# tongxyh/ImageCompression_Adversarial

Hardware: AMD Instinct MI355X
Metric: attack-step·images/sec, Balle2018-hyper 768×512 1001-step PGD, 1/2/4/8 GPU (higher is better)
Workload: dtype f32 (fp32-accurate: exact 3-way bf16 operand splits, 6 MFMA products, f32 accumulate); 1 GPU; attack_rd -m hyper -q 3 -att_metric L2 -noise 1e-4, 32 images/GPU of 768x512, steps of the 1001-step loop, x6 conv operands; per_gpu_batch=32, global_batch=32, height=512, width=768, parallelism=image-shard x1 (no data-path collective)

## Files before the change

imagecompression_adversarial_amd/_lib.py:

```python
from __future__ import annotations

import ctypes as C
import os

import torch

_HERE = os.path.dirname(os.path.abspath(__file__))
LIB_PATH = os.environ.get("ICA_HIP_LIB", os.path.join(_HERE, "libica_hip.so"))

_p = C.c_void_p
_i = C.c_int
_l = C.c_long
_f = C.c_float
_sz = C.c_size_t

_SIGS = {
    "ica_conv_it": [_i],
    "ica_pack_conv_weight_size": [_i, _i, _i, _i, _i],
    "ica_pack_conv_weight": [_p, _p, _i, _i, _i, _l, _l, _i, _i, _i, _i, _p],
    "ica_pack_conv_weight_bf16": [_p, _p, _i, _i, _i, _l, _l, _i, _i, _i, _p],
    "ica_pack_conv_weight_bf16_size": [_i, _i, _i, _i],
    "ica_pack_conv_weight_x6": [_p, _p, _i, _i, _i, _l, _l, _i, _i, _p],
    "ica_pack_conv_weight_x6_size": [_i, _i, _i, _i],
    "ica_pack_gdn_x6": [_p, _p, _i, _p],
    "ica_pack_gdn_x6_size": [_i],
    "ica_pack_up3_bf16": [_p, _p, _i, _p],
    "ica_pack_up3_x6": [_p, _p, _i, _p],
    "ica_pack_up3k3_x6_size": [_i],
    "ica_pack_up3k3_x6": [_p, _p, _p, _i, _p],
    "ica_conv_up3k3_x6": [_p, _p, _p, _p, _i, _i, _i, _i, _i, _i, _p],
    "ica_conv_up3_x6": [_p, _p, _p, _p, _i, _i, _i, _i, _i, _p],
    "ica_conv_up3_bf16": [_p, _p, _p, _p, _i, _i, _i, _i, _i, _p],
    "ica_conv_ex": [_p, _p],
    "ica_last_launch": [_p, _i, _p],
    "ica_pack_gdn": [_p, _p, _p, _p, _i, _i, _f, _p],
    "ica_pack_gdn_bf16": [_p, _p, _p, _p, _i, _i, _f, _p],
    "ica_pack_up3_size": [_i],
    "ica_pack_up3": [_p, _p, _i, _p],
    "ica_conv_up3": [_p, _p, _p, _p, _i, _i, _i, _i, _i, _p],
    "ica_elem_blocks_per_image": [],
    "ica_nchw_to_nc4": [_p, _p, _i, _i, _i, _i, _p],
    "ica_nc4_to_nchw": [_p, _p, _i, _i, _i, _i, _p],
    "ica_reduce_rows": [_p, _p, _i, _i, _f, _p],
    "ica_attack_prologue": [_p, _p, _p, _p, _i, _i, _i, _f, _p],
    "ica_attack_prologue_ex": [_p, _p, _p, _p, _i, _i, _i, _f, _i, _p],
    "ica_attack_loss": [_p, _p, _p, _p, _i, _i, _i, _f, _i, _i, _p],
    "ica_attack_adam": [_p, _p, _p, _p, _p, _p, _p, _p, _i, _i, _i, _f, _f, _f, _f, _f, _p, _p, _p, _p],
    "ica_attack_adam_ex": [_p, _p, _p, _p, _p, _p, _p, _p, _i, _i, _i, _f, _f, _f, _f, _f, _p, _p, _p, _i, _p],
# ... 73 lines not shown
    "ica_eb_bwd": [_p, _p, _p, _p, _p, _i, _i, _i, _i, _p],
    "ica_eb_param_scatter": [_p, _p, _p, _i, _p],
    "ica_mse_grad": [_p, _p, _p, _i, _i, _i, _f, _p],
}
_RESTYPES = {"ica_pack_conv_weight_size": _sz, "ica_pack_conv_weight_bf16_size": _sz,
             "ica_pack_conv_weight_x6_size": _sz, "ica_pack_gdn_x6_size": _sz, "ica_pack_up3k3_x6_size": _sz, "ica_pack_up3_size": _sz, "ica_wgrad_ws_size": _sz,
             "ica_rans_encode": _l, "ica_ar_lds_bytes": _sz, "ica_patch_vi_ws_size": _sz,
             "ica_gauss_blur_ws_size": _sz, "ica_blur_sweep_ws_size": _sz, "ica_noise_apply_ws_size": _sz}



class ConvArgs(C.Structure):
    _fields_ = ([(n, C.c_void_p) for n in ("x", "y", "wp", "bias", "gp", "beta", "save_x", "save_s", "in_x", "in_s",
                                            "save_t", "res", "mask")]
                + [(n, C.c_int) for n in ("N", "Cin", "Hin", "Win", "Cout", "Hout", "Wout", "kind", "KS", "S", "epi",
                                           "it", "fill_mode", "ps", "prec", "layout", "order")])


class ArArgs(C.Structure):
    _fields_ = ([(n, C.c_void_p) for n in ("y", "params", "yhat", "sym", "idx", "sym_in", "means", "wc", "bc", "w1",
                                            "b1", "w2", "b2", "w3", "b3", "table")]
                + [("T", C.c_int), ("bound", C.c_float)]
                + [(n, C.c_int) for n in ("B", "M", "H", "W", "E1", "E2")])


_lib = None


def lib():
    global _lib
    if _lib is None:
# ... 32 lines not shown
```

imagecompression_adversarial_amd/csrc/ica_conv.hip:

```cpp
#include <cxxabi.h>

#include <algorithm>
#include <cstdio>
#include <cstdlib>
#include <type_traits>

#include "ica_conv_epi.h"

#define ICA_WLOAD_BF(w, it, g) ((w)[(it) * 64])

template <int IT, int KH>
ICA_DEV void load_frag(float (&a)[IT][KH], const float* w) {
#pragma unroll
  for (int it = 0; it < IT; ++it) {
    if constexpr (KH == 8) {
      const f32x4 w0 = ld4(w + it * 64 * KH), w1 = ld4(w + it * 64 * KH + 4);
#pragma unroll
      for (int e = 0; e < 4; ++e) {
        a[it][e] = w0[e];
        a[it][4 + e] = w1[e];
      }
    } else {
      const f32x2 w0 = *reinterpret_cast<const f32x2*>(w + it * 64 * KH);
      a[it][0] = w0[0];
// ... 1381 lines not shown
              o2 += zs[(2 * 25 + tap) * NPX + q];
            }
          o[px] = f32x4{o0 + bias0, o1 + bias1, o2 + bias2, 0.f};
        }
        const int y = 2 * a + py, x = 2 * b;
        float* dst = p.y + (((size_t)n * p.Hout + y) * p.Wout + x) * 4;
        if (y < p.Hout) {
          st4(dst, o[0]);
          if (x + 1 < p.Wout) st4(dst + 4, o[1]);
        }
      }
    }
  }
}

__global__ void pack_up3_x6_kernel(const float* __restrict__ w, __bf16* __restrict__ dst, int Cin, long total) {
  const long i = (long)blockIdx.x * blockDim.x + threadIdx.x;
  if (i >= total) return;
  const int nch = Cin / 16;
  long t = i;
  const int s = t % 8; t /= 8;
  const int lane = t % 64; t /= 64;
  const int ch = t % nch; t /= nch;
  const int row = (int)t * 32 + (lane & 31);
  const int c = ch * 16 + (lane >> 5) * 8 + s;
  float v = 0.f;
  if (row < T3_ROWS) v = w[((size_t)c * 3 + row / 25) * 25 + row % 25];
  const __bf16 a = (__bf16)v;
  const float r1 = v - (float)a;
  const __bf16 b = (__bf16)r1;
// ... 454 lines not shown
  const float* bias;
  const float* gp;
  const float* beta;
  float* save_x;
  float* save_s;
  const float* in_x;
  const float* in_s;
  float* save_t;
  const float* res;
  const float* mask;
  int N, Cin, Hin, Win, Cout, Hout, Wout;
  int kind, KS, S, epi, it, fill_mode, ps;
  int prec;
  int layout;
  int order;
} ica_conv_args;

int ica_conv_it(int cout) {
  if (cout <= 32) return 1;
  if (cout % 128 == 0) return 4;
  if (cout % 96 == 0) return 3;
  return 4;
}

static inline int resolve_it(int O, int it) { return it > 0 ? it : ica_conv_it(O); }

size_t ica_pack_conv_weight_size(int O, int C, int KS, int CC, int it) {
  const int IT = resolve_it(O, it);
  const int ncb = (O + IT * 32 - 1) / (IT * 32);
  const int C4 = (C + 3) / 4, nch = (C4 * 4 + CC - 1) / CC;
// ... 106 lines not shown
               N, Cin, Hin, Win, 3, 2 * Hin, 2 * Win, nullptr};
  p.pl = layout;
  auto persistent = [&](auto kern, int R) {
    const int tiles = ((Win + U3_OW - 1) / U3_OW) * ((Hin + R - 1) / R) * N;
    const int nb = std::max(1, std::min((tiles + 7) / 8, ica_cu_count() / 8));
    ICA_LAUNCH(kern, dim3(8 * nb), dim3(256), 0, st, p);
  };
  if (Cin == 128) {
    persistent(conv_up3_x6p_kernel<8, 3>, u3_rows<3>());
  } else if (Cin == 192) {
    persistent(conv_up3_x6p_kernel<12, 2>, u3_rows<2>());
  } else {
    const int tiles = ((Win + T3_TW - 1) / T3_TW) * ((Hin + T3_TH - 1) / T3_TH) * N;
    ICA_LAUNCH((conv_up3_kernel<false, true>), dim3(tiles), dim3(256), 0, st, p);
  }
  ICA_CHECK_LAUNCH();
  return 0;
}

int ica_pack_up3_bf16(const float* w, void* dst, int Cin, hipStream_t st) {
  if (Cin % 16 != 0) return -2;
  const long total = (long)ica_pack_up3_size(Cin);
  ICA_LAUNCH(pack_up3_kernel<__bf16>, dim3((total + 255) / 256), dim3(256), 0, st, w,
                     reinterpret_cast<__bf16*>(dst), Cin, total);
  ICA_CHECK_LAUNCH();
  return 0;
}

int ica_conv_up3_bf16(const float* x, float* y, const void* wp, const float* bias, int N, int Cin, int Hin, int Win,
                      int layout, hipStream_t st) {
// ... 63 lines not shown
                     transpose, beta_bound);
  ICA_CHECK_LAUNCH();
  return 0;
}

int ica_conv_ex(const ica_conv_args* a, hipStream_t st) {
  ConvParams p{a->x,    a->y,    a->wp,   a->bias, a->gp,   a->beta, a->save_x, a->save_s, a->in_x, a->in_s,
               a->N,    a->Cin,  a->Hin,  a->Win,  a->Cout, a->Hout, a->Wout,   a->save_t, a->res,  a->mask,
               a->fill_mode, a->ps, a->prec, a->layout};
  if (a->prec < 0 || a->prec > 3) return -4;
  if (a->layout & ~(PL_IN | PL_OUT)) return -4;
  if (a->layout && (a->KS != 5 || a->S != 2 || a->fill_mode != 0 || a->ps)) return -4;
  if (((a->layout & PL_IN) && ((a->Hin | a->Win) & 1)) || ((a->layout & PL_OUT) && ((a->Hout | a->Wout) & 1)))
    return -2;
  const int it = resolve_it(a->Cout, a->it);
  if (a->epi >= EPI_GDN && a->epi <= EPI_IGDN_BWD && a->Cout != it * 32) return -4;
  if (a->ps && (a->Cout % 16 != 0 || !(a->epi == EPI_BIAS || a->epi == EPI_RELU || a->epi == EPI_LRELU))) return -4;
  if (a->fill_mode == 1 && !a->mask) return -4;
  if (a->fill_mode == 2 && a->Cin % 16 != 0) return -2;
  if (a->epi == EPI_LRELU_BWD && !a->in_x) return -4;
  const int fx = ((a->res || a->save_x) ? FX_RES : 0) | (a->ps ? FX_PS : 0) | (a->fill_mode == 1 ? FX_MASK : 0) |
                 (a->fill_mode == 2 ? FX_UNSHUF : 0) | (a->save_t ? FX_T : 0);
  const int want = a->kind == 1 ? ORDER_UP : ORDER_DOWN;
  if (a->prec == 2) {
    if (a->kind == 0 && a->KS == 3)
      return a->order == want ? pick_x6o<3>(p, a->kind, a->KS, a->S, a->epi, it, fx, st) : -4;
    return ica_conv_x6_dispatch(p, a->kind, a->KS, a->S, it, a->epi, fx, a->order, st);
  }
  if (a->prec == 3) return a->order == want ? pick_x6o<1>(p, a->kind, a->KS, a->S, a->epi, it, fx, st) : -4;
  if (a->prec == 1 && a->order == ORDER_RGB5) {
// ... 13 lines not shown
```

imagecompression_adversarial_amd/csrc/ica_conv_epi.h:

```cpp
#pragma once
#include "ica_common.h"

#ifndef ICA_X6_IEEE_GDN
#define ICA_X6_IEEE_GDN 0
#endif

enum {
  EPI_BIAS = 0,
  EPI_RELU = 1,
  EPI_GDN = 2,
  EPI_IGDN = 3,
  EPI_GDN_BWD = 4,
  EPI_IGDN_BWD = 5,
  EPI_LRELU = 6,
  EPI_LRELU_BWD = 7,
};
enum { FX_RES = 1, FX_PS = 2, FX_MASK = 4, FX_UNSHUF = 8, FX_T = 16 };

struct ConvParams {
  const float* x;
  float* y;
  const float* wp;
  const float* bias;
  const float* gp;
  const float* beta;
  float* save_x;
  float* save_s;
  const float* in_x;
  const float* in_s;
  int N, Cin, Hin, Win, Cout, Hout, Wout;
  float* save_t;
  const float* res;
  const float* mask;
  int fill_mode;
  int ps;
  int prec;
  int pl;
};
enum { PL_IN = 1, PL_OUT = 2 };
enum { ORDER_DOWN = 0, ORDER_UP = 1, ORDER_RGB5 = 2, ORDER_TG = 3 };

ICA_DEV void split3(f32x4 v, u32x2& hi, u32x2& mid, u32x2& lo) {
  bf16x4 a, b, c;
#pragma unroll
  for (int e = 0; e < 4; ++e) {
    const __bf16 h = (__bf16)v[e];
    const float r1 = v[e] - (float)h;
    const __bf16 m = (__bf16)r1;
    const float r2 = r1 - (float)m;
    a[e] = h;
    b[e] = m;
    c[e] = (__bf16)r2;
// ... 55 lines not shown
      v[i] = __builtin_bit_cast(f32x4, __builtin_amdgcn_raw_buffer_load_b128(grs, k * 2048 + l * 16, 0, 0));
    } else {
      v[i] = f32x4{0.f, 0.f, 0.f, 0.f};
    }
  }
#pragma unroll
  for (int i = 0; i < NI; ++i) {
    const int e = threadIdx.x + 256 * i;
    if (e < NP + NG) lp[e] = v[i];
  }
}

ICA_DEV unsigned pix_at(int y, int x, int H, int W, bool split) {
  return split ? ((unsigned)((((y & 1) << 1) | (x & 1)) * (H >> 1) + (y >> 1))) * (unsigned)(W >> 1) + (x >> 1)
               : (unsigned)y * W + x;
}

template <int IT, int EPI, int FX, bool BF = false, int X6 = 0, bool LG = false, int EAG = 1>
ICA_DEV void conv_epilogue(const ConvParams& p, f32x16 (&acc)[IT], int n, int oy, int ox,
                           bool valid, int co_base, const f32x4* lp = nullptr, float* lst = nullptr) {
  const int lane = threadIdx.x & 63, h = lane >> 5;
  const int C4o = (p.Cout + 3) >> 2;
  const unsigned plane = (unsigned)p.Hout * p.Wout;
  const unsigned pix = valid ? pix_at(oy, ox, p.Hout, p.Wout, p.pl & PL_OUT) : 0u;
  const size_t img = (size_t)C4o * plane;
  using Img = Img4T<BF>;
  const unsigned vo = h * plane + pix;
  auto so = [&](int u) -> unsigned { return (unsigned)u * plane; };
  const int cu = co_base >> 2;

// ... 299 lines not shown
          for (int s = 0; s < 2; ++s)
            uacc = mfma32bf(LG ? f4_as_bf8(lp[16 * IT + (k0 + s) * 64 + lane]) : ld_bf8(grs, lane * 16, o + s * 2048),
                            th[ct][s], uacc);
        }
        if (valid) {
#pragma unroll
          for (int g = 0; g < 4; ++g) {
            const f32x4 x2 = bf4_to_f4(x2q[jt][g]);
            f32x4 v;
#pragma unroll
            for (int e = 0; e < 4; ++e) v[e] = acc[jt][4 * g + e] + x2[e] * uacc[4 * g + e];
            Y.st(vo, so(jt * 8 + 2 * g), v);
          }
        }
      }
    } else if constexpr (FX == 0 && IT <= 4) {
      f32x16 tt[X6 == 1 ? 1 : IT], xx[IT];
      bf16x8 tq[X6 == 1 ? IT : 1][2][3];
      const unsigned vo_ld = valid ? vo : 0x0FFFFFF0u;
      float tw[8];
      __builtin_amdgcn_sched_barrier(0);
      f32x4 yq[X6 ? IT : 1][4], sq[X6 ? IT : 1][4];
      if constexpr (X6 != 0) {
#pragma unroll
        for (int it = 0; it < IT; ++it)
#pragma unroll
          for (int g = 0; g < 4; ++g) {
            yq[it][g] = IX.ld(vo_ld, so(it * 8 + 2 * g));
            sq[it][g] = IS.ld(vo_ld, so(it * 8 + 2 * g));
          }
        __builtin_amdgcn_sched_barrier(0);
// ... 38 lines not shown
#pragma unroll
          for (int jt = 0; jt < IT; ++jt)
#pragma unroll
            for (int q = 0; q < 3; ++q)
              a[jt][q] = ld_bf8(grs, lane * 16, (((jt * IT + (k >> 1)) * 2 + (k & 1)) * 1024) + q * IT * IT * 2048);
        };
        ldg(ga[0], 0);
#pragma unroll
        for (int k = 0; k < 2 * IT; ++k) {
          if (k + 1 < 2 * IT) ldg(ga[(k + 1) & 1], k + 1);
          __builtin_amdgcn_sched_barrier(0);
#pragma unroll
          for (int jt = 0; jt < IT; ++jt) ux[jt] = mfma_x6(ga[k & 1][jt], tq[k >> 1][k & 1], ux[jt]);
        }
      }
#pragma unroll
      for (int jt = 0; jt < IT; ++jt) {
        __builtin_amdgcn_sched_barrier(0);
        f32x16 uacc = f32x16{0};
#pragma unroll
        for (int ct = 0; ct < IT; ++ct) {
          if constexpr (X6 == 1) {
            if (ct == 0) uacc = ux[jt];
          } else if constexpr (X6 == 2) {
            if (ct % (IT / 2) == 0) {
              const __amdgpu_buffer_rsrc_t grs = uniform_rsrc(p.gp, IT * IT * 6144);
#pragma unroll
              for (int c2 = 0; c2 < IT / 2; ++c2)
#pragma unroll
                for (int s = 0; s < 2; ++s)
// ... 472 lines not shown
```

imagecompression_adversarial_amd/csrc/ica_conv_x6.hip:

```cpp
#include <algorithm>
#include <type_traits>

#include "ica_conv_epi.h"

namespace {

constexpr int X6_PT = 2;
constexpr int XD_TW = 32;
template <int PT>
constexpr int xd_th() { return 4 * PT; }

template <int IT, int EPI, int PT = X6_PT>
__global__ __launch_bounds__(256, 1) void conv_down_x6_kernel(ConvParams p, long ps) {
  ICA_STAMP_BEGIN();
  constexpr int KS = 5, S = 2, PAD = 2, KK = 25, TW = XD_TW, TH = xd_th<PT>();
  constexpr int PR = S * (TH - 1) + KS, PC = S * (TW - 1) + KS, PLANE = PR * PC;
  constexpr int NF = (4 * PLANE + 255) / 256, NB = (NF + 1) / 2;
  __shared__ f32x4 patch[3 * 2 * PLANE];
  const int tiles_x = (p.Wout + TW - 1) / TW, tiles_y = (p.Hout + TH - 1) / TH;
  int bid, cb;
  xcd_block<true>(bid, cb);
  const int tx = bid % tiles_x;
  bid /= tiles_x;
  const int ty = bid % tiles_y;
// ... 2062 lines not shown
  const int total = ((p.Wout + 31) / 32) * p.Hout * p.N;
  const int nblk = std::max(1, std::min(ica_cu_count(), (total + 7) / 8));
  constexpr int lds = rgb5b_lds_bytes<EPI>();
  static_assert(lds <= 160 * 1024, "conv_rgb5_bf16 LDS");
  static bool attr_set = false;
  if (!attr_set) {
    (void)hipFuncSetAttribute(reinterpret_cast<const void*>(&conv_rgb5_bf16_kernel<EPI>),
                              hipFuncAttributeMaxDynamicSharedMemorySize, lds);
    attr_set = true;
  }
  ICA_LAUNCH((conv_rgb5_bf16_kernel<EPI>), dim3(nblk), dim3(512), lds, st, p, nblk);
  ICA_CHECK_LAUNCH();
  return 0;
}

template <int IT, int EPI, int CG, int PT>
int launch_up_x6_pt(const ConvParams& p, hipStream_t st) {
  const int tiles = ((p.Win + XU_TW - 1) / XU_TW) * ((p.Hin + xu_th<PT>() - 1) / xu_th<PT>()) * p.N;
  const int ncb = (p.Cout + IT * 32 - 1) / (IT * 32);
  const long ps = (long)ncb * 25 * (p.Cin / 16) * IT * 64;
  constexpr size_t lds = xu_lds_bytes<CG, PT>();
  static_assert(lds <= 160 * 1024, "conv_up_x6 channel group exceeds LDS");
  static bool attr_set = false;
  if (!attr_set) {
    (void)hipFuncSetAttribute(reinterpret_cast<const void*>(&conv_up_x6_kernel<IT, EPI, CG, PT>),
                              hipFuncAttributeMaxDynamicSharedMemorySize, 160 * 1024);
    attr_set = true;
  }
  ICA_LAUNCH((conv_up_x6_kernel<IT, EPI, CG, PT>), dim3(tiles, ncb), dim3(256), lds, st, p, ps);
  ICA_CHECK_LAUNCH();
  return 0;
}

template <int IT, int EPI, int CG, int PT = 2>
int launch_up_x6w(const ConvParams& p, hipStream_t st) {
  const int tiles = ((p.Win + XU_TW - 1) / XU_TW) * ((p.Hin + xu_th<PT>() - 1) / xu_th<PT>()) * p.N;
  const int ncb = (p.Cout + IT * 32 - 1) / (IT * 32);
  const long ps = (long)ncb * 25 * (p.Cin / 16) * IT * 64;
  constexpr bool BWD = EPI == EPI_GDN_BWD || EPI == EPI_IGDN_BWD;
  constexpr size_t slabs = BWD ? (size_t)8 * 4 * IT * 64 * sizeof(f32x4) : 0;
  constexpr size_t lds = std::max((size_t)xu_lds_bytes<CG, PT>(), slabs);
  static_assert(lds <= 160 * 1024, "conv_up_x6w LDS");
  static bool attr_set = false;
  if (!attr_set) {
// ... 19 lines not shown
  constexpr bool BWD = EPI == EPI_GDN_BWD || EPI == EPI_IGDN_BWD;
#ifdef ICA_UPW_BWD_ALL
  constexpr bool SLAB = BWD && IT == 4;
#else
  constexpr bool SLAB = BWD && IT == 4 && CG == 64;
#endif
  if (x6_round_fill(b1) > x6_round_fill(b2) + 0.15) {
    if constexpr (SLAB) return launch_up_x6w<IT, EPI, CG, 1>(p, st);
    return launch_up_x6_pt<IT, EPI, CG, 1>(p, st);
  }
  if constexpr (SLAB) return launch_up_x6w<IT, EPI, CG, 2>(p, st);
  if constexpr (IT == 4 && !BWD) return launch_up_x6w<IT, EPI, CG>(p, st);
  return launch_up_x6_pt<IT, EPI, CG, X6_PT>(p, st);
}

template <int IT, int FX, int CG, int PT, int KS = 3>
int launch_up3s2_x6_pt(const ConvParams& p, hipStream_t st) {
  const int tiles = ((p.Win + XU_TW - 1) / XU_TW) * ((p.Hin + xu_th<PT>() - 1) / xu_th<PT>()) * p.N;
  const int ncb = (p.Cout + IT * 32 - 1) / (IT * 32);
  const long ps = (long)ncb * KS * KS * (p.Cin / 16) * IT * 64;
  constexpr size_t lds = xu_lds_bytes<CG, PT>();
  static_assert(lds <= 160 * 1024, "conv_up_x6 channel group exceeds LDS");
  static bool attr_set = false;
  if (!attr_set) {
    (void)hipFuncSetAttribute(reinterpret_cast<const void*>(&conv_up_x6_kernel<IT, EPI_BIAS, CG, PT, KS, FX>),
                              hipFuncAttributeMaxDynamicSharedMemorySize, 160 * 1024);
    attr_set = true;
  }
  ICA_LAUNCH((conv_up_x6_kernel<IT, EPI_BIAS, CG, PT, KS, FX>), dim3(tiles, ncb), dim3(256), lds, st, p, ps);
  ICA_CHECK_LAUNCH();
// ... 71 lines not shown
  return 0;
}

int ica_conv_x6_dispatch(const ConvParams& p, int kind, int KS, int S, int it, int epi, int fx, int order,
                         hipStream_t st) {
  const bool rgb = kind == 0 && KS == 5 && S == 2 && p.Cin <= 4;
  if (order != (rgb ? ORDER_RGB5 : kind == 1 ? ORDER_UP : ORDER_DOWN)) return -4;
  if (kind == 1 && KS == 3 && S == 2) return pick_up3s2_x6(p, it, epi, fx, st);
  if (kind == 1 && KS == 1 && S == 2) {
    if (epi != EPI_BIAS || fx != 0 || p.Cout % 32 != 0) return -4;
    if (p.Hout != 2 * p.Hin || p.Wout != 2 * p.Win || (p.pl & (PL_IN | PL_OUT))) return -2;
    if (it == 6 && p.Cin == 192) return launch_up3s2_x6_pt<6, 0, 192, 1, 1>(p, st);
    if (it == 4 && p.Cin == 128) return launch_up3s2_x6_pt<4, 0, 128, 2, 1>(p, st);
    return -3;
  }
  if (KS != 5 || S != 2 || fx != 0) return -4;
  if (p.Cout % 32 != 0) return -4;
  if (kind == 0) {
    if (p.Hout * 2 != p.Hin + (p.Hin & 1) || p.Wout * 2 != p.Win + (p.Win & 1)) return -2;
    if (p.Cin <= 4) {
      if (it != 4 || p.Cin > 3) return -3;
      if (p.pl & PL_IN) return -2;
      switch (epi) {
        case EPI_BIAS: return launch_rgb_x6<EPI_BIAS>(p, st);
        case EPI_GDN: return launch_rgb_x6<EPI_GDN>(p, st);
        case EPI_IGDN_BWD: return launch_rgb_x6<EPI_IGDN_BWD>(p, st);
        default: return -5;
      }
    }
    if (p.Cin < 16) return -2;
// ... 95 lines not shown
```

imagecompression_adversarial_amd/engine.py:

```python
from __future__ import annotations

import torch

from . import hip_ops as K


def _P(sd, prefix, name):
    return sd[f"{prefix}.{name}" if prefix else name]


class Saved(list):

    def __init__(self, items=(), split=(False,) * 5, exact=True):
        super().__init__(items)
        self.split = tuple(split)
        self.exact = exact


def _layout_of(saved):
    if not isinstance(saved, Saved):
        raise TypeError("backward needs the forward's Saved record (keep its type when selecting rows)")
    return saved.split


# ... 39 lines not shown
            p = self.convs[i]
            h, sx, ss = K.conv_down(h, C, p.fwd, p.bias, self.N, 5, 2, K.EPI_GDN, self.gdns[i], save,
                                    tag=f"{self.tag}.{2 * i}.fwd", layout=_lay(lv, i, i + 1))
            saved.append((sx, ss))
            C = self.N
        p = self.convs[3]
        y, _, _ = K.conv_down(h, self.N, p.fwd, p.bias, self.M, 5, 2, K.EPI_BIAS, tag=f"{self.tag}.6.fwd",
                              layout=_lay(lv, 3, 4))
        return y, saved

    def backward(self, gy4, saved):
        lv = _layout_of(saved)
        if not saved.exact:
            raise ValueError("g_a input gradient: image sides must be multiples of 16")
        g, C = gy4, self.M
        for i in (3, 2, 1):
            g, _, _ = K.conv_up(g, C, self.convs[i].bwd, None, self.N, K.EPI_GDN_BWD, self.gdns[i - 1],
                                saved=saved[i - 1], tag=f"{self.tag}.{2 * i}.dgrad", layout=_lay(lv, i + 1, i))
            C = self.N
        gx, _, _ = K.conv_up(g, self.N, self.convs[0].bwd, None, 3, K.EPI_BIAS, tag=f"{self.tag}.0.dgrad",
                             layout=_lay(lv, 1, 0))
        return gx


class Synthesis:

    def __init__(self, sd: dict, prefix: str = "g_s", tag: str = "g_s", prec: int = K.PREC_FP32):
        self.tag = tag
        self.M = _P(sd, prefix, "0.weight").shape[0]
        self.N = _P(sd, prefix, "0.weight").shape[1]
        g6 = 6 if self.N == 192 else 0
        self.convs = [K.PackedConv(_P(sd, prefix, f"{i}.weight"), _P(sd, prefix, f"{i}.bias"), "deconv", 2, prec,
                                   it_fwd=g6 if i < 6 else 0, it_bwd=g6 if i > 0 else 0)
                      for i in (0, 2, 4, 6)]
# ... 187 lines not shown
```

imagecompression_adversarial_amd/hip_ops.py:

```python
from __future__ import annotations

import math

import torch

from ._lib import ConvArgs, call, lib, ptr, stream

EPI_BIAS, EPI_RELU, EPI_GDN, EPI_IGDN, EPI_GDN_BWD, EPI_IGDN_BWD, EPI_LRELU, EPI_LRELU_BWD = range(8)
FILL_PLAIN, FILL_LRELU_MASK, FILL_UNSHUFFLE = range(3)
ORDER_DOWN, ORDER_UP = 0, 1
ORDER_RGB5 = 2
ORDER_TG = 3
ORDER_UP3 = 4
_ORDER_NAME = ("DOWN", "UP", "RGB5", "TG", "UP3")
LAYOUT_IN, LAYOUT_OUT = 1, 2
GDN_BETA_BOUND = float((1e-6 + 2.0 ** -36) ** 0.5)


EVENT_HOOK = None


def _ev_begin(tag, n):
    if EVENT_HOOK is None or tag is None:
        return None
# ... 325 lines not shown
        return _conv3(x4, Cin, wp, bias, Cout, 5, 2, 1, epi, gdn, save, saved, out, tag, save_t, layout, prec, it)
    _check_pack(wp, Cin, 3, 5, 1, prec, it)
    if wp.order != ORDER_UP3:
        raise ValueError(f"conv_up to 3 channels reads the Z-gather pack (ORDER_UP3), not {wp!r}")
    if epi != EPI_BIAS:
        raise RuntimeError("conv_up to 3 channels supports the bias epilogue only")
    N, _, H, W, _ = x4.shape
    y = out if out is not None else empty_nc4(N, 3, 2 * H, 2 * W, x4.device)
    ev = _ev_begin(_prec_note(tag, wp.prec), N)
    call({PREC_BF16: "ica_conv_up3_bf16", PREC_X6: "ica_conv_up3_x6"}.get(wp.prec, "ica_conv_up3"), ptr(x4), ptr(y),
         ptr(wp.data), ptr(bias), N, Cin, H, W, int(layout), stream())
    _ev_end(ev)
    return y, None, None


def conv_ex(x4, Cin, wp: Pack, bias, Cout, KS, S, kind=0, epi=EPI_BIAS, gdn: PackedGDN | None = None, res=None,
            save_x=None, save_s=None, saved=None, save_t=None, mask=None, fill_mode=FILL_PLAIN, ps=False,
            out=None, tag=None, alg_rows=None, layout=0, prec=None, it=0, _flops=True):
    _check_pack(wp, Cin, Cout, KS, kind, prec, it)
    if wp.order == ORDER_UP3:
        raise ValueError(f"{wp!r} is launched by conv_up to 3 channels only")
    if wp.order == ORDER_RGB5 and (epi not in (EPI_BIAS, EPI_GDN, EPI_IGDN_BWD) or fill_mode != FILL_PLAIN or ps
                                   or any(t is not None for t in (res, save_x, save_t, mask))):
        raise ValueError(f"{wp!r}: the dense tap-row pack is read by conv_rgb5 only (bias / GDN / IGDN_BWD epilogue, "
                         f"plain fill, no extra tensors)")
    prec = wp.prec
    N, C4x, H, W, _ = x4.shape
    if fill_mode == FILL_UNSHUFFLE:
        if Cin != 16 * C4x:
            raise RuntimeError("unshuffled conv input: Cin must be 16 * input channel groups")
        H, W = H // 2, W // 2
    Ho, Wo = _out_hw(H, W, KS, S, kind)
    dt = torch.bfloat16 if prec == PREC_BF16 else torch.float32
    if out is not None:
        y = out
    elif ps:
        y = torch.empty((N, Cout // 16, 2 * Ho, 2 * Wo, 4), dtype=dt, device=x4.device)
    else:
        y = empty_nc4(N, Cout, Ho, Wo, x4.device, dt)
    in_x = in_s = None
    if saved is not None:
        in_x, in_s = saved
    gp = None
    if gdn is not None:
        if prec == PREC_BF16:
            gdn.bf16()
            gp = gdn.gpbT if epi in (EPI_GDN_BWD, EPI_IGDN_BWD) else gdn.gpb
        elif prec in (PREC_X6, PREC_B1):
            gdn.x6()
            gp = gdn.gpxT if epi in (EPI_GDN_BWD, EPI_IGDN_BWD) else gdn.gpx
        else:
            gp = gdn.gpT if epi in (EPI_GDN_BWD, EPI_IGDN_BWD) else gdn.gp
    a = ConvArgs(ptr(x4), ptr(y), ptr(wp.data), ptr(bias), ptr(gp), ptr(None if gdn is None else gdn.beta),
                 ptr(save_x), ptr(save_s), ptr(in_x), ptr(in_s), ptr(save_t), ptr(res), ptr(mask), N, Cin, H, W, Cout,
                 Ho, Wo, kind, KS, S, epi, wp.it, fill_mode, int(bool(ps)), prec, int(layout), wp.order)
    import ctypes
    tag = _prec_note(tag, prec)
    ev = _ev_begin(tag, N)
    call("ica_conv_ex", ctypes.c_void_p(ctypes.addressof(a)), stream())
    if ev is not None:
        fl = None
        if _flops:
            px = N * (H * W if kind == 1 else Ho * Wo)
            cin_alg = alg_rows if (fill_mode == FILL_UNSHUFFLE and alg_rows) else Cin
            cout_alg = alg_rows if (ps and alg_rows) else Cout
            fl = 2.0 * cin_alg * cout_alg * KS * KS * px
            if epi in (EPI_GDN, EPI_IGDN, EPI_GDN_BWD, EPI_IGDN_BWD):
                fl += 2.0 * Cout * Cout * N * Ho * Wo
        _ev_end(ev, fl)
    return y
# ... 197 lines not shown
```

include/ica_hip.h:

```cpp
#ifndef ICA_HIP_H
#define ICA_HIP_H

#include <stddef.h>
#include <stdint.h>

#ifdef __cplusplus
extern "C" {
#endif

typedef struct ihipStream_t* hipStream_t;

enum { ICA_EPI_BIAS = 0, ICA_EPI_RELU = 1, ICA_EPI_GDN = 2, ICA_EPI_IGDN = 3, ICA_EPI_GDN_BWD = 4, ICA_EPI_IGDN_BWD = 5 };

int ica_conv_it(int cout);
size_t ica_pack_conv_weight_size(int O, int C, int KS, int CC, int it);
int ica_pack_conv_weight(const float* w, float* dst, int O, int C, int KS, long so, long sc, int CC, int order,
                         int flip, int it, hipStream_t stream);
int ica_pack_gdn(const float* gamma, const float* beta, float* gp, float* beta_eff, int C, int transpose,
                 float beta_bound, hipStream_t stream);
int ica_pack_conv_weight_bf16(const float* w, void* dst, int O, int C, int KS, long so, long sc, int order,
                              int flip, int it, hipStream_t stream);
int ica_pack_gdn_bf16(const float* gamma, const float* beta, void* gpb, float* beta_eff, int C, int transpose,
                      float beta_bound, hipStream_t stream);
int ica_pack_conv_weight_x6(const float* w, void* dst, int O, int C, int KS, long so, long sc, int order, int it,
// ... 51 lines not shown
  const float* wc;
  const float* bc;
  const float* w1;
  const float* b1;
  const float* w2;
  const float* b2;
  const float* w3;
  const float* b3;
  const float* table;
  int T;
  float bound;
  int B, M, H, W, E1, E2;
} ica_ar_args;
size_t ica_ar_lds_bytes(int M, int E1, int E2);
int ica_ar_step(const ica_ar_args* args, int p0, int p1, int mode, hipStream_t stream);
enum { ICA_EPI_LRELU = 6, ICA_EPI_LRELU_BWD = 7 };
enum { ICA_ORDER_DOWN = 0, ICA_ORDER_UP = 1, ICA_ORDER_RGB5 = 2, ICA_ORDER_TG = 3, ICA_ORDER_UP3 = 4 };
typedef struct ica_conv_args {
  const float* x;
  float* y;
  const float* wp;
  const float* bias;
  const float* gp;
  const float* beta;
  float* save_x;
  float* save_s;
  const float* in_x;
  const float* in_s;
  float* save_t;
  const float* res;
  const float* mask;
  int N, Cin, Hin, Win, Cout, Hout, Wout;
  int kind, KS, S, epi, it, fill_mode, ps;
  int prec;
  int layout;
  int order;
} ica_conv_args;
int ica_conv_ex(const ica_conv_args* args, hipStream_t stream);
int ica_last_launch(char* name, int cap, unsigned long long* threads);
size_t ica_pack_up3_size(int Cin);
int ica_pack_up3(const float* w, float* dst, int Cin, hipStream_t stream);
int ica_conv_up3(const float* x, float* y, const float* wp, const float* bias, int N, int Cin, int Hin, int Win,
                 int layout, hipStream_t stream);

int ica_elem_blocks_per_image(void);
int ica_nchw_to_nc4(const float* src, float* dst, int N, int C, int H, int W, hipStream_t stream);
int ica_nc4_to_nchw(const float* src, float* dst, int N, int C, int H, int W, hipStream_t stream);
int ica_reduce_rows(const float* part, float* out, int B, int nblk, float scale, hipStream_t stream);
int ica_attack_prologue(const float* noise, const float* im_s, float* im_in4, float* part, int B, int H, int W,
                        float eps, hipStream_t stream);
int ica_attack_prologue_ex(const float* noise, const float* im_s, float* im_in4, float* part, int B, int H, int W,
                           float eps, int clamp_in, hipStream_t stream);
int ica_attack_loss(const float* xhat4, const float* out_s, float* grad4, float* part, int B, int H, int W,
// ... 108 lines not shown
```

Measured before the change: 1539 attack-step·images/s.

## Fuse final 3-channel dgrad into GDN-backward conv epilogue via Z-gather

The last g_a input-gradient layer (128→3 channels, 5x5 stride-2 transposed) is folded into the epilogue of the preceding GDN-backward conv. After the GDN backward, the epilogue multiplies the 128-channel gradient by the packed 3-channel weights with x6 MFMAs and writes 75 per-tap partial planes Z. A new gather kernel then sums the taps into the 3-channel output and adds the bias. This avoids writing and re-reading the 128-channel intermediate and skips a separate low-occupancy conv. In exchange it adds a 75-plane fp32 scratch tensor, extra register pressure in the epilogue, and scattered stores.

```diff
diff --git a/imagecompression_adversarial_amd/_lib.py b/imagecompression_adversarial_amd/_lib.py
--- a/imagecompression_adversarial_amd/_lib.py
+++ b/imagecompression_adversarial_amd/_lib.py
@@ -32,6 +32,7 @@
     "ica_conv_up3_x6": [_p, _p, _p, _p, _i, _i, _i, _i, _i, _p],
     "ica_conv_up3_bf16": [_p, _p, _p, _p, _i, _i, _i, _i, _i, _p],
     "ica_conv_ex": [_p, _p],
+    "ica_zgather": [_p, _p, _p, _i, _i, _i, _p],
     "ica_last_launch": [_p, _i, _p],
     "ica_pack_gdn": [_p, _p, _p, _p, _i, _i, _f, _p],
     "ica_pack_gdn_bf16": [_p, _p, _p, _p, _i, _i, _f, _p],
@@ -135,7 +136,8 @@
     _fields_ = ([(n, C.c_void_p) for n in ("x", "y", "wp", "bias", "gp", "beta", "save_x", "save_s", "in_x", "in_s",
                                             "save_t", "res", "mask")]
                 + [(n, C.c_int) for n in ("N", "Cin", "Hin", "Win", "Cout", "Hout", "Wout", "kind", "KS", "S", "epi",
-                                           "it", "fill_mode", "ps", "prec", "layout", "order")])
+                                           "it", "fill_mode", "ps", "prec", "layout", "order")]
+                + [("wz", C.c_void_p)])
 
 
 class ArArgs(C.Structure):
diff --git a/imagecompression_adversarial_amd/csrc/ica_conv.hip b/imagecompression_adversarial_amd/csrc/ica_conv.hip
--- a/imagecompression_adversarial_amd/csrc/ica_conv.hip
+++ b/imagecompression_adversarial_amd/csrc/ica_conv.hip
@@ -1419,6 +1419,52 @@
   }
 }
 
+__global__ __launch_bounds__(256) void zgather_kernel(const float* __restrict__ z, float* __restrict__ y,
+                                                       const float* __restrict__ bias, int N, int Hin, int Win) {
+  const int W2 = Win >> 1, H2 = Hin >> 1, M4 = W2 >> 2;
+  const long idx = (long)blockIdx.x * 256 + threadIdx.x;
+  if (idx >= (long)N * Hin * M4 * 2) return;
+  const int pb = (int)(idx & 1);
+  long t = idx >> 1;
+  const int m = (int)(t % M4);
+  t /= M4;
+  const int a = (int)(t % Hin), n = (int)(t / Hin);
+  const size_t plane = (size_t)Hin * Win;
+  const float* zp = z + (size_t)n * T3_ROWS * plane + ((size_t)(((a & 1) << 1) | pb) * H2 + (a >> 1)) * W2 + 4 * m;
+  const float bias0 = bias ? bias[0] : 0.f, bias1 = bias ? bias[1] : 0.f, bias2 = bias ? bias[2] : 0.f;
+  const int Hout = 2 * Hin, Wout = 2 * Win;
+#pragma unroll
+  for (int py = 0; py < 2; ++py) {
+    float* row = y + ((size_t)n * Hout + 2 * a + py) * Wout * 4;
+#pragma unroll
+    for (int px = 0; px < 2; ++px) {
+      f32x4 o0 = {0.f, 0.f, 0.f, 0.f}, o1 = o0, o2 = o0;
+#pragma unroll
+      for (int ky = py; ky < 5; ky += 2)
+#pragma unroll
+        for (int kx = px; kx < 5; kx += 2) {
+          const int tap = ky * 5 + kx;
+          const bool rows_in = ky < 2 ? a + 1 < Hin : (ky < 4 || a > 0);
+          const int cut = kx < 2 ? (pb == 1 && m == M4 - 1 ? 3 : -1) : (kx == 4 && pb == 0 && m == 0 ? 0 : -1);
+          auto term = [&](int c) {
+            f32x4 v = ld4(zp + (c * 25 + tap) * plane);
+#pragma unroll
+            for (int i = 0; i < 4; ++i) v[i] = (!rows_in || i == cut) ? 0.f : v[i];
+            return v;
+          };
+          o0 += term(0);
+          o1 += term(1);
+          o2 += term(2);
+        }
+#pragma unroll
+      for (int i = 0; i < 4; ++i) {
+        const int x = 2 * (2 * (4 * m + i) + pb) + px;
+        st4(row + (size_t)x * 4, f32x4{o0[i] + bias0, o1[i] + bias1, o2[i] + bias2, 0.f});
+      }
+    }
+  }
+}
+
 __global__ void pack_up3_x6_kernel(const float* __restrict__ w, __bf16* __restrict__ dst, int Cin, long total) {
   const long i = (long)blockIdx.x * blockDim.x + threadIdx.x;
   if (i >= total) return;
@@ -1903,6 +1949,7 @@
   int prec;
   int layout;
   int order;
+  const float* wz;
 } ica_conv_args;
 
 int ica_conv_it(int cout) {
@@ -2039,6 +2086,14 @@
     const int tiles = ((Win + T3_TW - 1) / T3_TW) * ((Hin + T3_TH - 1) / T3_TH) * N;
     ICA_LAUNCH((conv_up3_kernel<false, true>), dim3(tiles), dim3(256), 0, st, p);
   }
+  ICA_CHECK_LAUNCH();
+  return 0;
+}
+
+int ica_zgather(const float* z, float* y, const float* bias, int N, int Hin, int Win, hipStream_t st) {
+  if (N <= 0 || Hin <= 0 || Win <= 0 || (Hin & 1) || (Win & 7)) return -2;
+  const long items = (long)N * Hin * (Win >> 3) * 2;
+  ICA_LAUNCH(zgather_kernel, dim3((unsigned)((items + 255) / 256)), dim3(256), 0, st, z, y, bias, N, Hin, Win);
   ICA_CHECK_LAUNCH();
   return 0;
 }
@@ -2132,6 +2187,13 @@
   if (((a->layout & PL_IN) && ((a->Hin | a->Win) & 1)) || ((a->layout & PL_OUT) && ((a->Hout | a->Wout) & 1)))
     return -2;
   const int it = resolve_it(a->Cout, a->it);
+  if (a->epi == EPI_GDN_BWD_Z) {
+    if (a->prec != 2 || a->kind != 1 || a->KS != 5 || a->S != 2 || !a->wz || a->order != ORDER_UP || a->res ||
+        a->save_x || a->save_t || a->ps || a->fill_mode != 0 || a->Cout != 128 || it != 4 || !a->in_x || !a->in_s)
+      return -4;
+    p.wz = a->wz;
+    return ica_conv_x6_dispatch(p, 1, 5, 2, 4, EPI_GDN_BWD, FX_Z, a->order, st);
+  }
   if (a->epi >= EPI_GDN && a->epi <= EPI_IGDN_BWD && a->Cout != it * 32) return -4;
   if (a->ps && (a->Cout % 16 != 0 || !(a->epi == EPI_BIAS || a->epi == EPI_RELU || a->epi == EPI_LRELU))) return -4;
   if (a->fill_mode == 1 && !a->mask) return -4;
diff --git a/imagecompression_adversarial_amd/csrc/ica_conv_epi.h b/imagecompression_adversarial_amd/csrc/ica_conv_epi.h
--- a/imagecompression_adversarial_amd/csrc/ica_conv_epi.h
+++ b/imagecompression_adversarial_amd/csrc/ica_conv_epi.h
@@ -14,8 +14,9 @@
   EPI_IGDN_BWD = 5,
   EPI_LRELU = 6,
   EPI_LRELU_BWD = 7,
+  EPI_GDN_BWD_Z = 8,
 };
-enum { FX_RES = 1, FX_PS = 2, FX_MASK = 4, FX_UNSHUF = 8, FX_T = 16 };
+enum { FX_RES = 1, FX_PS = 2, FX_MASK = 4, FX_UNSHUF = 8, FX_T = 16, FX_Z = 32 };
 
 struct ConvParams {
   const float* x;
@@ -36,6 +37,7 @@
   int ps;
   int prec;
   int pl;
+  const float* wz;
 };
 enum { PL_IN = 1, PL_OUT = 2 };
 enum { ORDER_DOWN = 0, ORDER_UP = 1, ORDER_RGB5 = 2, ORDER_TG = 3 };
@@ -121,6 +123,75 @@
 ICA_DEV unsigned pix_at(int y, int x, int H, int W, bool split) {
   return split ? ((unsigned)((((y & 1) << 1) | (x & 1)) * (H >> 1) + (y >> 1))) * (unsigned)(W >> 1) + (x >> 1)
                : (unsigned)y * W + x;
+}
+
+constexpr int Z_ROWS = 75, Z_NCH = 8;
+ICA_DEV constexpr int z_shift(int k) { return k < 2 ? 1 : k < 4 ? 0 : -1; }
+ICA_DEV constexpr int z_dy(int row) { return row < Z_ROWS ? z_shift((row % 25) / 5) : 0; }
+ICA_DEV constexpr int z_dx(int row) { return row < Z_ROWS ? z_shift(row % 5) : 0; }
+
+template <int IT>
+ICA_DEV void gdn_bwd_z_store(const ConvParams& p, f32x16 (&acc)[IT], int n, int oy, int ox, bool valid) {
+  static_assert(IT * 2 == Z_NCH, "128 channels");
+  const int lane = threadIdx.x & 63, h = lane >> 5;
+  constexpr long pst = 3L * Z_NCH * 64;
+  const __amdgpu_buffer_rsrc_t wr = uniform_rsrc(p.wz, (unsigned)(3 * pst * 16));
+  auto ldw = [&](bf16x8 (&a)[3][3], int ch) {
+#pragma unroll
+    for (int it = 0; it < 3; ++it)
+#pragma unroll
+      for (int q = 0; q < 3; ++q) a[it][q] = ld_bf8(wr, lane * 16, (int)((q * pst + ((long)it * Z_NCH + ch) * 64) * 16));
+  };
+  f32x16 za[3];
+#pragma unroll
+  for (int it = 0; it < 3; ++it) za[it] = f32x16{0};
+  bf16x8 wa[2][3][3];
+  ldw(wa[0], 0);
+#pragma unroll
+  for (int ch = 0; ch < Z_NCH; ++ch) {
+    if (ch + 1 < Z_NCH) ldw(wa[(ch + 1) & 1], ch + 1);
+    __builtin_amdgcn_sched_barrier(0);
+    const int jt = ch >> 1, s = ch & 1;
+    float v[8];
+#pragma unroll
+    for (int e = 0; e < 4; ++e) {
+      const float q0 = acc[jt][8 * s + e], q1 = acc[jt][8 * s + 4 + e];
+      const float got = __shfl_xor(h ? q0 : q1, 32, 64);
+      v[e] = h ? got : q0;
+      v[4 + e] = h ? q1 : got;
+    }
+    bf16x8 b[3];
+    split3x8(v, b);
+#pragma unroll
+    for (int it = 0; it < 3; ++it) za[it] = mfma_x6(wa[ch & 1][it], b, za[it]);
+  }
+  __builtin_amdgcn_sched_barrier(0);
+  const unsigned plane = (unsigned)p.Hout * p.Wout;
+  const __amdgpu_buffer_rsrc_t zr =
+      uniform_rsrc(reinterpret_cast<const char*>(p.y) + (size_t)n * Z_ROWS * plane * 4, Z_ROWS * plane * 4u);
+  constexpr unsigned ZOOB = 0xC0000000u;
+  unsigned po[3][3];
+#pragma unroll
+  for (int sy = 0; sy < 3; ++sy)
+#pragma unroll
+    for (int sx = 0; sx < 3; ++sx) {
+      const int ya = oy - (sy - 1), xb = ox - (sx - 1);
+      const bool ok = valid && ya >= 0 && ya < p.Hout && xb >= 0 && xb < p.Wout;
+      po[sy][sx] = ok ? pix_at(ok ? ya : 0, ok ? xb : 0, p.Hout, p.Wout, true) * 4u : ZOOB;
+    }
+  const unsigned plane4 = plane * 4u;
+#pragma unroll
+  for (int it = 0; it < 3; ++it)
+#pragma unroll
+    for (int r = 0; r < 16; ++r) {
+      const int r0 = it * 32 + acc_row(r, 0), r1 = it * 32 + acc_row(r, 1);
+      if (r0 < Z_ROWS) {
+        const unsigned o0 = po[z_dy(r0) + 1][z_dx(r0) + 1] + (unsigned)r0 * plane4;
+        const unsigned o1 = r1 < Z_ROWS ? po[z_dy(r1) + 1][z_dx(r1) + 1] + (unsigned)r1 * plane4 : ZOOB;
+        const float zv = za[it][r];
+        __builtin_amdgcn_raw_buffer_store_b32(__builtin_bit_cast(unsigned, zv), zr, (int)(h ? o1 : o0), 0, 0);
+      }
+    }
 }
 
 template <int IT, int EPI, int FX, bool BF = false, int X6 = 0, bool LG = false, int EAG = 1>
@@ -450,7 +521,8 @@
           }
         }
       }
-    } else if constexpr (FX == 0 && IT <= 4) {
+    } else if constexpr ((FX & ~FX_Z) == 0 && IT <= 4) {
+      static_assert((FX & FX_Z) == 0 || (X6 == 1 && IT == 4), "Z epilogue: the wide x6 form, 128 channels");
       f32x16 tt[X6 == 1 ? 1 : IT], xx[IT];
       bf16x8 tq[X6 == 1 ? IT : 1][2][3];
       const unsigned vo_ld = valid ? vo : 0x0FFFFFF0u;
@@ -519,6 +591,14 @@
           for (int jt = 0; jt < IT; ++jt) ux[jt] = mfma_x6(ga[k & 1][jt], tq[k >> 1][k & 1], ux[jt]);
         }
       }
+      if constexpr ((FX & FX_Z) != 0) {
+#pragma unroll
+        for (int jt = 0; jt < IT; ++jt)
+#pragma unroll
+          for (int r = 0; r < 16; ++r) acc[jt][r] = acc[jt][r] + xx[jt][r] * ux[X6 == 1 ? jt : 0][r];
+        __builtin_amdgcn_sched_barrier(0);
+        gdn_bwd_z_store<IT>(p, acc, n, oy, ox, valid);
+      } else
 #pragma unroll
       for (int jt = 0; jt < IT; ++jt) {
         __builtin_amdgcn_sched_barrier(0);
diff --git a/imagecompression_adversarial_amd/csrc/ica_conv_x6.hip b/imagecompression_adversarial_amd/csrc/ica_conv_x6.hip
--- a/imagecompression_adversarial_amd/csrc/ica_conv_x6.hip
+++ b/imagecompression_adversarial_amd/csrc/ica_conv_x6.hip
@@ -2100,7 +2100,7 @@
   return 0;
 }
 
-template <int IT, int EPI, int CG, int PT>
+template <int IT, int EPI, int CG, int PT, int FX = 0>
 int launch_up_x6_pt(const ConvParams& p, hipStream_t st) {
   const int tiles = ((p.Win + XU_TW - 1) / XU_TW) * ((p.Hin + xu_th<PT>() - 1) / xu_th<PT>()) * p.N;
   const int ncb = (p.Cout + IT * 32 - 1) / (IT * 32);
@@ -2109,11 +2109,11 @@
   static_assert(lds <= 160 * 1024, "conv_up_x6 channel group exceeds LDS");
   static bool attr_set = false;
   if (!attr_set) {
-    (void)hipFuncSetAttribute(reinterpret_cast<const void*>(&conv_up_x6_kernel<IT, EPI, CG, PT>),
+    (void)hipFuncSetAttribute(reinterpret_cast<const void*>(&conv_up_x6_kernel<IT, EPI, CG, PT, 5, FX>),
                               hipFuncAttributeMaxDynamicSharedMemorySize, 160 * 1024);
     attr_set = true;
   }
-  ICA_LAUNCH((conv_up_x6_kernel<IT, EPI, CG, PT>), dim3(tiles, ncb), dim3(256), lds, st, p, ps);
+  ICA_LAUNCH((conv_up_x6_kernel<IT, EPI, CG, PT, 5, FX>), dim3(tiles, ncb), dim3(256), lds, st, p, ps);
   ICA_CHECK_LAUNCH();
   return 0;
 }
@@ -2163,6 +2163,15 @@
   return launch_up_x6_pt<IT, EPI, CG, X6_PT>(p, st);
 }
 
+static int launch_up_x6_z(const ConvParams& p, hipStream_t st) {
+  if (p.Cin != 128 || p.Cout != 128 || !p.wz || p.Hin * p.Win <= XS_SMALL_PX || ((p.Hout | p.Wout) & 1)) return -4;
+  if ((size_t)96 * p.Hout * p.Wout * 4 >= ((size_t)1 << 30)) return -2;
+  const long b2 = (long)((p.Win + XU_TW - 1) / XU_TW) * ((p.Hin + xu_th<2>() - 1) / xu_th<2>()) * p.N;
+  const long b1 = (long)((p.Win + XU_TW - 1) / XU_TW) * ((p.Hin + xu_th<1>() - 1) / xu_th<1>()) * p.N;
+  if (x6_round_fill(b1) > x6_round_fill(b2) + 0.15) return launch_up_x6_pt<4, EPI_GDN_BWD, 128, 1, FX_Z>(p, st);
+  return launch_up_x6_pt<4, EPI_GDN_BWD, 128, X6_PT, FX_Z>(p, st);
+}
+
 template <int IT, int FX, int CG, int PT, int KS = 3>
 int launch_up3s2_x6_pt(const ConvParams& p, hipStream_t st) {
   const int tiles = ((p.Win + XU_TW - 1) / XU_TW) * ((p.Hin + xu_th<PT>() - 1) / xu_th<PT>()) * p.N;
@@ -2264,6 +2273,10 @@
     if (it == 4 && p.Cin == 128) return launch_up3s2_x6_pt<4, 0, 128, 2, 1>(p, st);
     return -3;
   }
+  if (KS == 5 && S == 2 && fx == FX_Z) {
+    if (kind != 1 || it != 4 || epi != EPI_GDN_BWD || p.Hout != 2 * p.Hin || p.Wout != 2 * p.Win) return -4;
+    return launch_up_x6_z(p, st);
+  }
   if (KS != 5 || S != 2 || fx != 0) return -4;
   if (p.Cout % 32 != 0) return -4;
   if (kind == 0) {
diff --git a/imagecompression_adversarial_amd/engine.py b/imagecompression_adversarial_amd/engine.py
--- a/imagecompression_adversarial_amd/engine.py
+++ b/imagecompression_adversarial_amd/engine.py
@@ -77,10 +77,18 @@
         if not saved.exact:
             raise ValueError("g_a input gradient: image sides must be multiples of 16")
         g, C = gy4, self.M
-        for i in (3, 2, 1):
+        for i in (3, 2):
             g, _, _ = K.conv_up(g, C, self.convs[i].bwd, None, self.N, K.EPI_GDN_BWD, self.gdns[i - 1],
                                 saved=saved[i - 1], tag=f"{self.tag}.{2 * i}.dgrad", layout=_lay(lv, i + 1, i))
             C = self.N
+        N, _, H2, W2, _ = g.shape
+        if K.ZFUSE and K.zfuse_ok(self.convs[1].bwd, self.convs[0].bwd, H2, W2):
+            z = torch.empty((N, 75, 2 * H2, 2 * W2), device=g.device)
+            K.conv_up_z(g, self.convs[1].bwd, self.gdns[0], saved[0], self.convs[0].bwd, z,
+                        tag=f"{self.tag}.2.dgrad", layout=_lay(lv, 2, 1))
+            return K.zgather(z, tag=f"{self.tag}.0.dgrad")
+        g, _, _ = K.conv_up(g, C, self.convs[1].bwd, None, self.N, K.EPI_GDN_BWD, self.gdns[0],
+                            saved=saved[0], tag=f"{self.tag}.2.dgrad", layout=_lay(lv, 2, 1))
         gx, _, _ = K.conv_up(g, self.N, self.convs[0].bwd, None, 3, K.EPI_BIAS, tag=f"{self.tag}.0.dgrad",
                              layout=_lay(lv, 1, 0))
         return gx
diff --git a/imagecompression_adversarial_amd/hip_ops.py b/imagecompression_adversarial_amd/hip_ops.py
--- a/imagecompression_adversarial_amd/hip_ops.py
+++ b/imagecompression_adversarial_amd/hip_ops.py
@@ -1,12 +1,16 @@
 from __future__ import annotations
 
 import math
+import os
 
 import torch
 
 from ._lib import ConvArgs, call, lib, ptr, stream
 
 EPI_BIAS, EPI_RELU, EPI_GDN, EPI_IGDN, EPI_GDN_BWD, EPI_IGDN_BWD, EPI_LRELU, EPI_LRELU_BWD = range(8)
+EPI_GDN_BWD_Z = 8
+ZFUSE = os.environ.get("ICA_ZFUSE", "1") != "0"
+X6_SMALL_PX = 32 * 32
 FILL_PLAIN, FILL_LRELU_MASK, FILL_UNSHUFFLE = range(3)
 ORDER_DOWN, ORDER_UP = 0, 1
 ORDER_RGB5 = 2
@@ -363,9 +367,31 @@
     return y, None, None
 
 
+def zfuse_ok(wp: Pack, wz: Pack, H: int, W: int) -> bool:
+    return (wp.prec == PREC_X6 and wz.prec == PREC_X6 and wp.order == ORDER_UP and wz.order == ORDER_UP3
+            and (wp.O, wp.C, wp.KS, wp.it, wz.C) == (128, 128, 5, 4, 128) and H * W > X6_SMALL_PX and W % 4 == 0
+            and 96 * 16 * H * W < 2 ** 30)
+
+
+def conv_up_z(x4, wp: Pack, gdn: PackedGDN, saved, wz: Pack, z: torch.Tensor, tag=None, layout=0):
+    return conv_ex(x4, wp.C, wp, None, wp.O, 5, 2, 1, EPI_GDN_BWD_Z, gdn, saved=saved, out=z, tag=tag, layout=layout,
+                   _flops=False, wz=wz)
+
+
+def zgather(z: torch.Tensor, bias=None, out=None, tag=None):
+    N, R, H, W = z.shape
+    if R != 75 or z.dtype != torch.float32 or not z.is_contiguous():
+        raise ValueError("zgather reads a contiguous fp32 Z tensor [N, 75, H, W]")
+    y = out if out is not None else empty_nc4(N, 3, 2 * H, 2 * W, z.device)
+    ev = _ev_begin(_prec_note(tag, PREC_X6), N)
+    call("ica_zgather", ptr(z), ptr(y), ptr(bias), N, H, W, stream())
+    _ev_end(ev)
+    return y
+
+
 def conv_ex(x4, Cin, wp: Pack, bias, Cout, KS, S, kind=0, epi=EPI_BIAS, gdn: PackedGDN | None = None, res=None,
             save_x=None, save_s=None, saved=None, save_t=None, mask=None, fill_mode=FILL_PLAIN, ps=False,
-            out=None, tag=None, alg_rows=None, layout=0, prec=None, it=0, _flops=True):
+            out=None, tag=None, alg_rows=None, layout=0, prec=None, it=0, _flops=True, wz: Pack | None = None):
     _check_pack(wp, Cin, Cout, KS, kind, prec, it)
     if wp.order == ORDER_UP3:
         raise ValueError(f"{wp!r} is launched by conv_up to 3 channels only")
@@ -375,6 +401,13 @@
                          f"plain fill, no extra tensors)")
     prec = wp.prec
     N, C4x, H, W, _ = x4.shape
+    if (epi == EPI_GDN_BWD_Z) != (wz is not None):
+        raise ValueError("wz (the 3-channel layer's x6 Z-gather pack) goes with EPI_GDN_BWD_Z, and only with it")
+    if wz is not None:
+        if (wz.order, wz.prec, wz.O, wz.C, wz.KS) != (ORDER_UP3, PREC_X6, 3, Cout, 5) or prec != PREC_X6:
+            raise ValueError(f"EPI_GDN_BWD_Z multiplies by an x6 Z-gather pack of {Cout} channels, not {wz!r}")
+        if out is None or out.dtype != torch.float32 or tuple(out.shape) != (N, 75, 2 * H, 2 * W):
+            raise ValueError("EPI_GDN_BWD_Z writes a caller-held fp32 Z tensor [N, 75, 2H, 2W] (out=)")
     if fill_mode == FILL_UNSHUFFLE:
         if Cin != 16 * C4x:
             raise RuntimeError("unshuffled conv input: Cin must be 16 * input channel groups")
@@ -397,12 +430,13 @@
             gp = gdn.gpbT if epi in (EPI_GDN_BWD, EPI_IGDN_BWD) else gdn.gpb
         elif prec in (PREC_X6, PREC_B1):
             gdn.x6()
-            gp = gdn.gpxT if epi in (EPI_GDN_BWD, EPI_IGDN_BWD) else gdn.gpx
+            gp = gdn.gpxT if epi in (EPI_GDN_BWD, EPI_IGDN_BWD, EPI_GDN_BWD_Z) else gdn.gpx
         else:
             gp = gdn.gpT if epi in (EPI_GDN_BWD, EPI_IGDN_BWD) else gdn.gp
     a = ConvArgs(ptr(x4), ptr(y), ptr(wp.data), ptr(bias), ptr(gp), ptr(None if gdn is None else gdn.beta),
                  ptr(save_x), ptr(save_s), ptr(in_x), ptr(in_s), ptr(save_t), ptr(res), ptr(mask), N, Cin, H, W, Cout,
-                 Ho, Wo, kind, KS, S, epi, wp.it, fill_mode, int(bool(ps)), prec, int(layout), wp.order)
+                 Ho, Wo, kind, KS, S, epi, wp.it, fill_mode, int(bool(ps)), prec, int(layout), wp.order,
+                 ptr(None if wz is None else wz.data))
     import ctypes
     tag = _prec_note(tag, prec)
     ev = _ev_begin(tag, N)
diff --git a/include/ica_hip.h b/include/ica_hip.h
--- a/include/ica_hip.h
+++ b/include/ica_hip.h
@@ -89,7 +89,7 @@
 } ica_ar_args;
 size_t ica_ar_lds_bytes(int M, int E1, int E2);
 int ica_ar_step(const ica_ar_args* args, int p0, int p1, int mode, hipStream_t stream);
-enum { ICA_EPI_LRELU = 6, ICA_EPI_LRELU_BWD = 7 };
+enum { ICA_EPI_LRELU = 6, ICA_EPI_LRELU_BWD = 7, ICA_EPI_GDN_BWD_Z = 8 };
 enum { ICA_ORDER_DOWN = 0, ICA_ORDER_UP = 1, ICA_ORDER_RGB5 = 2, ICA_ORDER_TG = 3, ICA_ORDER_UP3 = 4 };
 typedef struct ica_conv_args {
   const float* x;
@@ -110,8 +110,10 @@
   int prec;
   int layout;
   int order;
+  const float* wz;
 } ica_conv_args;
 int ica_conv_ex(const ica_conv_args* args, hipStream_t stream);
+int ica_zgather(const float* z, float* y, const float* bias, int N, int Hin, int Win, hipStream_t stream);
 int ica_last_launch(char* name, int cap, unsigned long long* threads);
 size_t ica_pack_up3_size(int Cin);
 int ica_pack_up3(const float* w, float* dst, int Cin, hipStream_t stream);
```

Measured after the change: 1525 attack-step·images/s. No clear change (-0.9%).
